# bentherien/point-cloud-reid

Hardware: AMD Instinct MI355X
Metric: siamese pair-comparisons/sec @1024 pts (higher is better)
Workload: dtype bf16x3

## Files before the change

### point-cloud-reid_amd/csrc/attn_kernels_impl.h

```cpp
#pragma once
#ifndef PCR_ATTN_PREC
#define PCR_ATTN_PREC 0
#endif
#include "tile_dense.h"

#include <stdio.h>

#include <vector>

namespace {
constexpr int kAPrec = PCR_ATTN_PREC;
struct AttnArgs {
  pcr_attn_params p;
  int dbg;
  int wpc;
};

constexpr int kATraceWgs = 512, kATraceRecs = 24, kATraceMarks = 8;
__device__ unsigned long long g_attn_trace[2 * kATraceWgs * kATraceRecs * kATraceMarks];


__device__ __forceinline__ void pos_hidden(float *dst, int RP, const float *P, const float *w0,
                                           const float *b0, int d, int T) {
  for (int e = threadIdx.x; e < d * T; e += blockDim.x) {
// ... 636 lines not shown
        for (int s2 = 0; s2 < 2; s2++) {
          float xv[8];
#pragma unroll
          for (int e = 0; e < 8; e++) xv[e] = xf[8 * s2 + e];
          bf_split8(xv, ah[s2], al[s2], true);
        }
        f32x16 acc[2];
#pragma unroll
        for (int cb = 0; cb < 2; cb++)
#pragma unroll
          for (int r = 0; r < 16; r++) acc[cb][r] = 0.f;
        const bf16x8 *wb = reinterpret_cast<const bf16x8 *>(s_w) + lane;
#pragma unroll
        for (int s2 = 0; s2 < 4; s2++) {
          bf16x8 wh[2], wl[2];
#pragma unroll
          for (int cb = 0; cb < 2; cb++) {
            wh[cb] = wb[((s2 * 2 + cb) * 2) * 64];
            wl[cb] = wb[((s2 * 2 + cb) * 2 + 1) * 64];
          }
#pragma unroll
          for (int cb = 0; cb < 2; cb++) acc[cb] = __builtin_amdgcn_mfma_f32_32x32x16_bf16(ah[s2], wh[cb], acc[cb], 0, 0, 0);
#pragma unroll
          for (int cb = 0; cb < 2; cb++) acc[cb] = __builtin_amdgcn_mfma_f32_32x32x16_bf16(al[s2], wh[cb], acc[cb], 0, 0, 0);
#pragma unroll
          for (int cb = 0; cb < 2; cb++) acc[cb] = __builtin_amdgcn_mfma_f32_32x32x16_bf16(ah[s2], wl[cb], acc[cb], 0, 0, 0);
        }
#pragma unroll
        for (int r = 0; r < 16; r++) {
          acc[0][r] = elu1(acc[0][r] + bias0);
          acc[1][r] = (acc[1][r] + bias1) * inv_sk;
          ks += acc[0][r];
        }
#pragma unroll
        for (int r = 0; r < 16; r++) kv = __builtin_amdgcn_mfma_f32_32x32x2f32(acc[0][r], acc[1][r], kv, 0, 0, 0);
      }
    }
    ks += __shfl_xor(ks, 32, 64);
    float *KVl = s_red + cslot * KVS, *s_kt = KVl + D * LD;
    for (int round = 0; round < wpc2; round++) {
      if (wsub == round) {
#pragma unroll
        for (int r = 0; r < 16; r++) {
          float *dst = KVl + ((r & 3) + 8 * (r >> 2) + 4 * h) * LD + j;
          *dst = round == 0 ? kv[r] : *dst + kv[r];
        }
        if (h == 0) s_kt[j] = round == 0 ? ks : s_kt[j] + ks;
      }
      __syncthreads();
    }
    if (live && wsub == 0) {
      float *kvo = p.kv + (size_t)b * ((size_t)D * D + D);
      const float *ap = s_wm + j * LD + h;
      const float *bp = KVl + j * LD + h;
      const int hd = j / dh;
      f32x16 m;
#pragma unroll
      for (int r = 0; r < 16; r++) m[r] = 0.f;
#pragma unroll 4
      for (int s2 = 0; s2 < 16; s2++) {
        const float bv = bp[2 * s2];
        m = __builtin_amdgcn_mfma_f32_32x32x2f32((2 * s2 + h) / dh == hd ? bv : 0.f, ap[2 * s2], m, 0, 0, 0);
      }
      bf16x8 *img = reinterpret_cast<bf16x8 *>(kvo);
#pragma unroll
      for (int G = 0; G < 2; G++) {
        float v[8];
#pragma unroll
        for (int e = 0; e < 8; e++) v[e] = m[8 * G + e];
        bf16x8 hi, lo;
        bf_split8(v, hi, lo, true);
        const size_t unit = (((size_t)G * (D >> 5)) * 2) * 64 + h * 32 + j;
        img[unit] = hi;
        img[unit + 64] = lo;
      }
      if (lane < D) kvo[(size_t)D * D + lane] = s_kt[lane];
    }
    __syncthreads();
  }
}
#endif

__global__ __launch_bounds__(kThreads) void attn_kv_fold_kernel(AttnArgs a) {
  extern __shared__ __attribute__((aligned(16))) float smem[];
  const pcr_attn_params &p = a.p;
  const int d = p.d, dh = d / p.nhead, ld = d + 1, nsplit = p.kv_splits, tid = threadIdx.x;
  const size_t b = blockIdx.x, per = (size_t)d * d + d;
  float *KVl = smem, *s_kt = smem + d * ld;
  const float *part = p.kv_part + b * nsplit * per;
  for (int e = tid; e < d * d + d; e += kThreads) {
    float v = part[e];
    for (int y = 1; y < nsplit; y++) v += part[(size_t)y * per + e];
    if (e < d * d) {
      const int dd = e / d, c = e - dd * d;
      KVl[dd * ld + c] = (dd / dh == c / dh) ? v : 0.f;
    } else {
      s_kt[e - d * d] = v;
    }
  }
  __syncthreads();
  attn_kv_fold_write(p, KVl, s_kt, b);
}

#if PCR_ATTN_PREC == 0
template <int NRW>
__global__ __launch_bounds__(kThreads) void attn_kv_wide_kernel(AttnArgs a) {
  constexpr int TB = 1, T = 32, RP = 33, BAND = 64, RPK = BAND + 1;
  extern __shared__ __attribute__((aligned(16))) float smem[];
  const pcr_attn_params &p = a.p;
  const int d = p.d, c2 = p.c2, dh = d / p.nhead;
  const int g = blockIdx.x, hd = (g * BAND) / dh;
  const int OPW = BAND + dh;
  float *XH = smem;
  float *KB = XH, *VB = XH + BAND * RP;
  float *P = XH + (c2 + d) * RP;
  float *s_w0 = P + 3 * RP, *s_b0 = s_w0 + 3 * d;
  float *s_ks = s_b0 + d;
  const int tid = threadIdx.x, lane = tid & 63, wave = tid >> 6;
  const int l31 = lane & 31, h = lane >> 5;
  const size_t b = blockIdx.y;
  for (int e = tid; e < 3 * d; e += kThreads) s_w0[e] = p.pos0_w[e];
  for (int e = tid; e < d; e += kThreads) s_b0[e] = p.pos0_b[e];
  const float *feat = p.feat_k + b * c2 * p.Sk;
  const float *xyz = p.xyz_k + b * p.Sk * 3;
  const float sk = (float)p.Sk;
  const float *wband = p.wkv_wide + (size_t)g * ((size_t)ceil8(c2 + d) * OPW);
  const float *bband = p.bkv_wide + (size_t)g * OPW;
  const int nj = dh >> 5, nT = 2 * nj;
  f32x16 acc[4];
#pragma unroll
  for (int i = 0; i < 4; i++)
#pragma unroll
    for (int r = 0; r < 16; r++) acc[i][r] = 0.f;
  const int krow = tid & (BAND - 1), kpart = tid >> 6;
  float ksum = 0.f;
  for (int t0 = 0; t0 < p.Sk; t0 += T) {
    const int valid = p.Sk - t0;
    load_tile(XH, RP, feat, c2, c2, p.Sk, t0, T);
    load_xyz3(P, RP, xyz, p.Sk, t0, T);
    __syncthreads();
    pos_hidden(XH + c2 * RP, RP, P, s_w0, s_b0, d, T);
    __syncthreads();
    tile_dense2<TB, NRW, 0, true>(XH, c2 + d, wband, OPW, true,
                                  [&](const f32x16 &acc, int cb, int tb, int l31, int h) {
      const int t = tb * 32 + l31;
      float *dst = XH + (cb * 32 + 4 * h) * RP + t;
      const bool live = t < valid;
      if (cb * 32 < BAND) {
#pragma unroll
        for (int r = 0; r < 16; r++) dst[((r & 3) + 8 * (r >> 2)) * RP] = live ? elu1(acc[r]) : 0.f;
      } else {
#pragma unroll
        for (int r = 0; r < 16; r++) dst[((r & 3) + 8 * (r >> 2)) * RP] = live ? acc[r] / sk : 0.f;
      }
    }, bband);
    __syncthreads();
    {
      const float *row = KB + krow * RP;
      for (int t = kpart; t < T; t += 4) ksum += row[t];
    }
#pragma unroll
    for (int it = 0; it < 4; it++) {
      const int item = wave + 4 * it;
      if (item < nT) {
        const int ib = item / nj, jb = item - ib * nj;
        const float *ap = KB + (ib * 32 + l31) * RP + h;
        const float *bp = VB + (jb * 32 + l31) * RP + h;
#pragma unroll 4
        for (int ks = 0; ks < T / 2; ks++)
          acc[it] = __builtin_amdgcn_mfma_f32_32x32x2f32(ap[2 * ks], bp[2 * ks], acc[it], 0, 0, 0);
      }
    }
    __syncthreads();
  }
  float *KVt = smem;
  s_ks[tid] = ksum;
  __syncthreads();
  const float ks_total = tid < BAND ? s_ks[tid] + s_ks[64 + tid] + s_ks[128 + tid] + s_ks[192 + tid] : 0.f;
  __syncthreads();
#pragma unroll
  for (int it = 0; it < 4; it++) {
    const int item = wave + 4 * it;
    if (item < nT) {
      const int ib = item / nj, jb = item - ib * nj;
      const int v = jb * 32 + l31;
#pragma unroll
      for (int r = 0; r < 16; r++) KVt[v * RPK + ib * 32 + (r & 3) + 8 * (r >> 2) + 4 * h] = acc[it][r];
    }
  }
  __syncthreads();
  float *kv = p.kv + b * ((size_t)d * d + d);
  if (tid < BAND) kv[(size_t)d * d + g * BAND + tid] = ks_total;
  const float *wm = p.wmerge_packed + (size_t)(hd * dh / 8) * d * 8;
  tile_dense(KVt, dh, RPK, 2, wm, d, [&](float m, int o, int t) {
    const int dd = g * BAND + t;
    const int kb = dd >> 3, rem = dd & 7;
    kv[(((size_t)kb * d + o) * 2 + (rem & 1)) * 4 + (rem >> 1)] = m;
  });
}

#endif

template <int TB, int NR>
__global__ __launch_bounds__(kThreads) void attn_apply_kernel(AttnArgs a) {
  constexpr int T = 32 * TB, RP = T + 1;
  extern __shared__ __attribute__((aligned(16))) float smem[];
  const pcr_attn_params &p = a.p;
  const int d = p.d, c1 = p.c1, cout = p.cout;
  const int catC = c1 + d, catP = ceil8(catC);
  int rowsU = catP > 2 * d ? catP : 2 * d;
  if (ceil32(cout) > rowsU) rowsU = ceil32(cout);
  if (ceil32(p.cfinal) > rowsU) rowsU = ceil32(p.cfinal);
  float *U = smem;
  float *P = U + rowsU * RP;
  float *zs = P + 3 * RP;
  float *red = zs + p.nhead * RP;
  float *cst = red + 2 * (kThreads / T) * T;
  float *s_ksum = cst, *s_ln1g = cst + d, *s_ln1b = cst + 2 * d, *s_ln2g = cst + 3 * d, *s_ln2b = s_ln2g + cout;
  float *s_w0 = s_ln2b + cout, *s_b0 = s_w0 + 3 * d;
  const int tid = threadIdx.x;
  const size_t b = blockIdx.y;
  const int t0 = blockIdx.x * T;
  const size_t bq_ = p.q_index ? (size_t)p.q_index[b] : b;
  const float *feat = p.feat_q + bq_ * c1 * p.Lq;
  const size_t kb_ = p.kv_index ? (size_t)p.kv_index[b] : b;
  const float *kv = p.kv + kb_ * ((size_t)d * d + d);
  const int dh = d / p.nhead;
  for (int e = tid; e < d; e += kThreads) {
    s_ksum[e] = kv[(size_t)d * d + e];
    s_ln1g[e] = p.ln1_g[e];
    s_ln1b[e] = p.ln1_b[e];
    if (p.q_pos) {
      s_w0[3 * e] = p.pos0_w[3 * e];
      s_w0[3 * e + 1] = p.pos0_w[3 * e + 1];
      s_w0[3 * e + 2] = p.pos0_w[3 * e + 2];
      s_b0[e] = p.pos0_b[e];
    }
  }
  for (int e = tid; e < cout; e += kThreads) {
    s_ln2g[e] = p.ln2_g[e];
    s_ln2b[e] = p.ln2_b[e];
  }
  const float *ksum = s_ksum;
  float *MSG = U + c1 * RP;

  load_tile(U, RP, feat, c1, c1, p.Lq, t0, T);
  if (p.q_pos) {
    load_xyz3(P, RP, p.xyz_q + bq_ * p.Lq * 3, p.Lq, t0, T);
    __syncthreads();
    pos_hidden(MSG, RP, P, s_w0, s_b0, d, T);
    for (int e = tid; e < (catP - catC) * T; e += kThreads) U[(catC + e / T) * RP + e % T] = 0.f;
  } else {
    for (int e = tid; e < (catP - c1) * T; e += kThreads) U[(c1 + e / T) * RP + e % T] = 0.f;
  }
  __syncthreads();
  tile_dense2p<kAPrec, TB, NR>(U, p.q_pos ? catP : ceil8(c1), p.wq, d, true,
                               [&](float v, int o, int t) { MSG[o * RP + t] = elu1(v); }, p.bq);
  __syncthreads();
  for (int e = tid; e < p.nhead * T; e += kThreads) {
    const int hd = e / T, t = e - hd * T;
    float z = 0.f;
    for (int c = 0; c < dh; c++) z += MSG[(hd * dh + c) * RP + t] * ksum[hd * dh + c];
    zs[hd * RP + t] = (1.0f / (z + 1e-6f)) * (float)p.Sk;
  }
  __syncthreads();
  for (int hd = 0; hd < p.nhead; hd++)
    for (int e = tid; e < dh * T; e += kThreads) {
      const int o = hd * dh + e / T, t = e % T;
      MSG[o * RP + t] *= zs[hd * RP + t];
    }
  __syncthreads();
  tile_dense2p<kAPrec, TB, NR>(MSG, d, kv, d, true, [&](float v, int o, int t) { MSG[o * RP + t] = v; });
  __syncthreads();
  tile_layernorm(MSG, d, RP, T, s_ln1g, s_ln1b, red);
  tile_dense2p<kAPrec, TB, NR>(U, catP, p.wmlp0, 2 * d, true, [&](float v, int o, int t) { U[o * RP + t] = fmaxf(v, 0.f); });
  __syncthreads();
  tile_dense2p<kAPrec, TB, NR>(U, 2 * d, p.wmlp2, ceil32(cout), true, [&](float v, int o, int t) { U[o * RP + t] = v; });
  __syncthreads();
  tile_layernorm(U, cout, RP, T, s_ln2g, s_ln2b, red);
  if (p.residual) {
    for (int e = tid; e < cout * T; e += kThreads) {
      const int c = e / T, t = e - c * T;
      if (t0 + t < p.Lq) U[c * RP + t] += feat[(size_t)c * p.Lq + t0 + t];
    }
    __syncthreads();
  }
  int cres = cout;
  if (p.cfinal) {
    const int cf = p.cfinal;
    tile_dense2p<kAPrec, TB, NR>(U, cout, p.wfinal, ceil32(cf), true, [&](float v, int o, int t) { U[o * RP + t] = v; },
                                 p.bfinal);
    __syncthreads();
    cres = cf;
  }
  float *out = p.out + b * cres * p.Lq;
  for (int e = tid; e < cres * T; e += kThreads) {
    const int c = e / T, t = e - c * T;
    if (t0 + t < p.Lq) out[(size_t)c * p.Lq + t0 + t] = U[c * RP + t];
  }
}

#if PCR_ATTN_PREC != 0
constexpr int kApsWaves = 8;
template <bool QPOS, int C1S, int CF, int NOB = 2, int ND = 2, bool POOL = false>
__global__ __launch_bounds__(64 * kApsWaves) __attribute__((amdgpu_waves_per_eu(2, 2)))
void attn_apply_stream64_kernel(AttnArgs a) {
  static_assert(!QPOS || C1S == 2 * ND, "q_pos needs c1 == d");
  static_assert(NOB <= 2 || (NOB == 4 && !CF), "cout = 128 has no trailing conv");
  static_assert(!POOL || (!CF && NOB == 2), "pooled output: cout = 64, no trailing conv");
  constexpr int D = 32 * ND, SD = 2 * ND;
  constexpr int SQ = C1S + (QPOS ? SD : 0), S0 = C1S + SD, NX = 8 * C1S;
  extern __shared__ __attribute__((aligned(16))) float smem[];
  const pcr_attn_params &p = a.p;
  bf16x8 *s_wq = reinterpret_cast<bf16x8 *>(smem);
  bf16x8 *s_w0 = s_wq + SQ * ND * 128;
  bf16x8 *s_w2 = s_w0 + S0 * ND * 256;
  float *s_c = reinterpret_cast<float *>(s_w2 + ND * NOB * 512);
  f32x4 *s_p0 = reinterpret_cast<f32x4 *>(s_c + 448);
  float *s_ks = reinterpret_cast<float *>(s_p0 + 64);
  const int tid = threadIdx.x, lane = tid & 63, j = lane & 31, h = lane >> 5;
  const int wave = __builtin_amdgcn_readfirstlane(tid >> 6);
  {
    const f32x4 *wq = reinterpret_cast<const f32x4 *>(p.wq),
                *w0 = reinterpret_cast<const f32x4 *>((p.c1 & 15) ? p.wmlp0_bf_xpad : p.wmlp0),
                *w2 = reinterpret_cast<const f32x4 *>(p.wmlp2);
    f32x4 *dq = reinterpret_cast<f32x4 *>(s_wq), *d0 = reinterpret_cast<f32x4 *>(s_w0), *d2 = reinterpret_cast<f32x4 *>(s_w2);
    for (int e = tid; e < SQ * ND * 128; e += 64 * kApsWaves) dq[e] = wq[e];
    for (int e = tid; e < S0 * ND * 256; e += 64 * kApsWaves) d0[e] = w0[e];
    for (int e = tid; e < ND * NOB * 512; e += 64 * kApsWaves) d2[e] = w2[e];
    if (tid < D) {
      s_c[tid] = p.bq[tid];
      s_c[64 + tid] = p.ln1_g[tid];
      s_c[128 + tid] = p.ln1_b[tid];

      if (QPOS) s_p0[tid] = f32x4{p.pos0_w[3 * tid], p.pos0_w[3 * tid + 1], p.pos0_w[3 * tid + 2], p.pos0_b[tid]};
    }
    if (tid < 32 * NOB) {
      s_c[192 + tid] = p.ln2_g[tid];
      s_c[192 + 32 * NOB + tid] = p.ln2_b[tid];
    }
    if (CF && tid < 32 * CF) s_c[320 + tid] = p.bfinal[tid];
  }
  __syncthreads();
  const int nblk = p.Lq >> 5;
  const long nitem = (long)p.B * nblk;
  const int dh = D / p.nhead;
  const float skf = (float)p.Sk;
  float *ksw = s_ks + wave * 64;
  auto cvec = [&](const float *base, int cb, int g) __attribute__((always_inline)) {
    return *reinterpret_cast<const f32x4 *>(base + 32 * cb + 8 * g + 4 * h);
  };
  auto to_ops = [&](const f32x16 &acc, int G, bf16x8 &oh, bf16x8 &ol) __attribute__((always_inline)) {
    float v[8];
#pragma unroll
    for (int e = 0; e < 8; e++) v[e] = acc[8 * G + e];
    bf_split8(v, oh, ol, true);
  };
#ifdef PCR_SA_TRACE_BUILD
  const bool tracing = (a.dbg & 256) && lane == 0 && (wave == 0 || wave == 5) && blockIdx.x < kATraceWgs;
  unsigned long long *trace = g_attn_trace + (size_t)(2 * blockIdx.x + (wave ? 1 : 0)) * (kATraceRecs * kATraceMarks);
  int trace_it = 0;
#define PCR_AMARK(m)                                                                                       \
  do {                                                                                                     \
    if (tracing && trace_it < kATraceRecs) trace[trace_it * kATraceMarks + (m)] = __builtin_readcyclecounter(); \
  } while (0)
#define PCR_ANEXT() trace_it++
#else
#define PCR_AMARK(m) do { } while (0)
#define PCR_ANEXT() do { } while (0)
#endif
  const long nwav = (long)gridDim.x * kApsWaves, gw = (long)blockIdx.x * kApsWaves + wave;
  long pc = gw;
  int pblk = 0;
  float pmax = -INFINITY, psum = 0.f;
  for (long it = gw; POOL ? pc < p.B : it < nitem; it += POOL ? 0 : nwav) {
    asm volatile("" ::: "memory");
    PCR_AMARK(0);
    const long b = POOL ? pc : it / nblk;
    const int blk = POOL ? pblk : (int)(it - b * nblk);
    const size_t bq_ = p.q_index ? (size_t)p.q_index[b] : (size_t)b;
    const size_t kb_ = p.kv_index ? (size_t)p.kv_index[b] : (size_t)b;
    const float *kvp = p.kv + kb_ * ((size_t)D * D + D);
    const int t = blk * 32 + j;
    const __amdgpu_buffer_rsrc_t rfeat = __builtin_amdgcn_make_buffer_rsrc(
        const_cast<float *>(p.feat_q + bq_ * p.c1 * p.Lq), 0, p.c1 * p.Lq * 4, 0x00020000);
    const int vo = (4 * h * p.Lq + t) * 4;
    float xf[NX];
#pragma unroll
    for (int e = 0; e < NX; e++) {
      const int ch = 16 * (e >> 3) + bf_kpos(0, e & 7);
      xf[e] = __builtin_bit_cast(float, __builtin_amdgcn_raw_buffer_load_b32(rfeat, vo, ch * p.Lq * 4, 0));
    }
    if (lane < D) ksw[lane] = kvp[(size_t)D * D + lane];
    bf16x8 bh[4 * ND], bl[4 * ND];
    if constexpr (QPOS) {
      const float *xyz = p.xyz_q + (bq_ * p.Lq + t) * 3;
      const float px = xyz[0], py = xyz[1], pz = xyz[2];
#pragma unroll
      for (int s2 = 0; s2 < SD; s2++) {
        float hv[8];
#pragma unroll
        for (int e = 0; e < 8; e++) {
          const f32x4 w = s_p0[16 * s2 + bf_kpos(0, e) + 4 * h];
          const float v = w[0] * px + w[1] * py + w[2] * pz + w[3];
          hv[e] = relu_i(v);
        }
        bf_split8(hv, bh[C1S + s2], bl[C1S + s2], true);
      }
    }
#pragma unroll
    for (int e = 0; e < NX; e++) asm volatile("" : "+v"(xf[e]));
#pragma unroll
    for (int s2 = 0; s2 < C1S; s2++) {
      float xv[8];
#pragma unroll
      for (int e = 0; e < 8; e++) xv[e] = xf[8 * s2 + e];
      bf_split8(xv, bh[s2], bl[s2], true);
    }
    PCR_AMARK(1);
    f32x16 q[ND];
#pragma unroll
    for (int cb = 0; cb < ND; cb++)
#pragma unroll
      for (int r = 0; r < 16; r++) q[cb][r] = 0.f;
    {
      const bf16x8 *wb = s_wq + lane;
#pragma unroll
      for (int s2 = 0; s2 < SQ; s2++) {
        bf16x8 wh[ND], wl[ND];
#pragma unroll
        for (int cb = 0; cb < ND; cb++) {
          wh[cb] = wb[((s2 * ND + cb) * 2) * 64];
          wl[cb] = wb[((s2 * ND + cb) * 2 + 1) * 64];
        }
#pragma unroll
        for (int cb = 0; cb < ND; cb++) q[cb] = __builtin_amdgcn_mfma_f32_32x32x16_bf16(wh[cb], bh[s2], q[cb], 0, 0, 0);
#pragma unroll
        for (int cb = 0; cb < ND; cb++) q[cb] = __builtin_amdgcn_mfma_f32_32x32x16_bf16(wh[cb], bl[s2], q[cb], 0, 0, 0);
#pragma unroll
        for (int cb = 0; cb < ND; cb++) q[cb] = __builtin_amdgcn_mfma_f32_32x32x16_bf16(wl[cb], bh[s2], q[cb], 0, 0, 0);
      }
    }
    PCR_AMARK(2);
    bf16x8 mh[SD][ND], ml[SD][ND];
    {
      const bf16x8 *mb = reinterpret_cast<const bf16x8 *>(kvp) + lane;
#pragma unroll
      for (int s2 = 0; s2 < SD; s2++)
#pragma unroll
        for (int cb = 0; cb < ND; cb++) {
          mh[s2][cb] = mb[((s2 * ND + cb) * 2) * 64];
          ml[s2][cb] = mb[((s2 * ND + cb) * 2 + 1) * 64];
        }
    }
    __builtin_amdgcn_fence(__ATOMIC_RELEASE, "wavefront");
    __builtin_amdgcn_wave_barrier();
    __builtin_amdgcn_fence(__ATOMIC_ACQUIRE, "wavefront");
    float z16[2][2] = {{0.f, 0.f}, {0.f, 0.f}};
#pragma unroll
    for (int cb = 0; cb < ND; cb++)
#pragma unroll
      for (int g = 0; g < 4; g++) {
        const f32x4 bqv = cvec(s_c, cb, g), ksv = cvec(ksw, cb, g);
        float zz = 0.f;
#pragma unroll
        for (int qq = 0; qq < 4; qq++) {
          const float v = elu1(q[cb][4 * g + qq] + bqv[qq]);
          q[cb][4 * g + qq] = v;
          zz += v * ksv[qq];
        }
        if ((g & 1) == 0) z16[cb][g >> 1] = zz;
        else z16[cb][g >> 1] += zz;
      }
    float zs[2][2];
    {
      float za = z16[0][0], zb = z16[0][1], zc = z16[1][0], zd = z16[1][1];
      if (dh >= 32) {
        za += zb; zb = za;
        zc += zd; zd = zc;
      }
      if (ND == 2 && dh >= 64) {
        za += zc; zb = za; zc = za; zd = za;
      }
      za += __shfl_xor(za, 32, 64);
      zb += __shfl_xor(zb, 32, 64);
      zc += __shfl_xor(zc, 32, 64);
      zd += __shfl_xor(zd, 32, 64);
      zs[0][0] = (1.0f / (za + 1e-6f)) * skf;
      zs[0][1] = (1.0f / (zb + 1e-6f)) * skf;
      zs[1][0] = (1.0f / (zc + 1e-6f)) * skf;
      zs[1][1] = (1.0f / (zd + 1e-6f)) * skf;
    }
#pragma unroll
    for (int cb = 0; cb < ND; cb++)
#pragma unroll
      for (int r = 0; r < 16; r++) q[cb][r] *= zs[cb][r >> 3];
    bf16x8 ch_[SD], cl_[SD];
#pragma unroll
    for (int cb = 0; cb < ND; cb++)
#pragma unroll
      for (int G = 0; G < 2; G++) to_ops(q[cb], G, ch_[2 * cb + G], cl_[2 * cb + G]);
    f32x16 m[ND];
#pragma unroll
    for (int cb = 0; cb < ND; cb++)
#pragma unroll
      for (int r = 0; r < 16; r++) m[cb][r] = 0.f;
#pragma unroll
    for (int s2 = 0; s2 < SD; s2++) {
#pragma unroll
      for (int cb = 0; cb < ND; cb++) m[cb] = __builtin_amdgcn_mfma_f32_32x32x16_bf16(mh[s2][cb], ch_[s2], m[cb], 0, 0, 0);
#pragma unroll
      for (int cb = 0; cb < ND; cb++) m[cb] = __builtin_amdgcn_mfma_f32_32x32x16_bf16(mh[s2][cb], cl_[s2], m[cb], 0, 0, 0);
#pragma unroll
      for (int cb = 0; cb < ND; cb++) m[cb] = __builtin_amdgcn_mfma_f32_32x32x16_bf16(ml[s2][cb], ch_[s2], m[cb], 0, 0, 0);
    }
    auto layernorm = [&](auto &v, auto nb_tag, const float *gam, const float *bet) __attribute__((always_inline)) {
      constexpr int NB = decltype(nb_tag)::value;
      float sm = 0.f;
#pragma unroll
      for (int cb = 0; cb < NB; cb++)
#pragma unroll
        for (int r = 0; r < 16; r++) sm += v[cb][r];
      sm += __shfl_xor(sm, 32, 64);
      const float mean = sm / (32.0f * NB);
      float vr = 0.f;
#pragma unroll
      for (int cb = 0; cb < NB; cb++)
#pragma unroll
        for (int r = 0; r < 16; r++) {
          const float dlt = v[cb][r] - mean;
          vr += dlt * dlt;
        }
      vr += __shfl_xor(vr, 32, 64);
      const float inv = 1.0f / sqrtf(vr / (32.0f * NB) + 1e-5f);
#pragma unroll
      for (int cb = 0; cb < NB; cb++)
#pragma unroll
        for (int g = 0; g < 4; g++) {
          const f32x4 gv = cvec(gam, cb, g), bv = cvec(bet, cb, g);
#pragma unroll
          for (int qq = 0; qq < 4; qq++) v[cb][4 * g + qq] = (v[cb][4 * g + qq] - mean) * inv * gv[qq] + bv[qq];
        }
    };
    PCR_AMARK(3);
    layernorm(m, std::integral_constant<int, ND>{}, s_c + 64, s_c + 128);
    PCR_AMARK(4);
#pragma unroll
    for (int s2 = 0; s2 < C1S; s2++) {
      float xv[8];
#pragma unroll
      for (int e = 0; e < 8; e++) xv[e] = xf[8 * s2 + e];
      bf_split8(xv, bh[s2], bl[s2], true);
    }
#pragma unroll
    for (int cb = 0; cb < ND; cb++)
#pragma unroll
      for (int G = 0; G < 2; G++) to_ops(m[cb], G, bh[C1S + 2 * cb + G], bl[C1S + 2 * cb + G]);
    f32x16 f[SD];
#pragma unroll
    for (int cb = 0; cb < SD; cb++)
#pragma unroll
      for (int r = 0; r < 16; r++) f[cb][r] = 0.f;
    {
      const bf16x8 *wb = s_w0 + lane;
#pragma unroll
      for (int s2 = 0; s2 < S0; s2++) {
        bf16x8 wh[SD], wl[SD];
#pragma unroll
        for (int cb = 0; cb < SD; cb++) {
          wh[cb] = wb[((s2 * SD + cb) * 2) * 64];
          wl[cb] = wb[((s2 * SD + cb) * 2 + 1) * 64];
        }
#pragma unroll
        for (int cb = 0; cb < SD; cb++) f[cb] = __builtin_amdgcn_mfma_f32_32x32x16_bf16(wh[cb], bh[s2], f[cb], 0, 0, 0);
#pragma unroll
        for (int cb = 0; cb < SD; cb++) f[cb] = __builtin_amdgcn_mfma_f32_32x32x16_bf16(wh[cb], bl[s2], f[cb], 0, 0, 0);
#pragma unroll
        for (int cb = 0; cb < SD; cb++) f[cb] = __builtin_amdgcn_mfma_f32_32x32x16_bf16(wl[cb], bh[s2], f[cb], 0, 0, 0);
      }
    }
#pragma unroll
    for (int cb = 0; cb < SD; cb++) {
#pragma unroll
      for (int r = 0; r < 16; r++) f[cb][r] = relu_i(f[cb][r]);
#pragma unroll
      for (int G = 0; G < 2; G++) to_ops(f[cb], G, bh[2 * cb + G], bl[2 * cb + G]);
    }
    PCR_AMARK(5);
    f32x16 o[NOB];
#pragma unroll
    for (int cb = 0; cb < NOB; cb++)
#pragma unroll
      for (int r = 0; r < 16; r++) o[cb][r] = 0.f;
    {
      const bf16x8 *wb = s_w2 + lane;
#pragma unroll
      for (int s2 = 0; s2 < 4 * ND; s2++) {
        bf16x8 wh[NOB], wl[NOB];
#pragma unroll
        for (int cb = 0; cb < NOB; cb++) {
          wh[cb] = wb[((s2 * NOB + cb) * 2) * 64];
          wl[cb] = wb[((s2 * NOB + cb) * 2 + 1) * 64];
        }
#pragma unroll
        for (int cb = 0; cb < NOB; cb++) o[cb] = __builtin_amdgcn_mfma_f32_32x32x16_bf16(wh[cb], bh[s2], o[cb], 0, 0, 0);
#pragma unroll
        for (int cb = 0; cb < NOB; cb++) o[cb] = __builtin_amdgcn_mfma_f32_32x32x16_bf16(wh[cb], bl[s2], o[cb], 0, 0, 0);
#pragma unroll
        for (int cb = 0; cb < NOB; cb++) o[cb] = __builtin_amdgcn_mfma_f32_32x32x16_bf16(wl[cb], bh[s2], o[cb], 0, 0, 0);
      }
    }
    PCR_AMARK(6);
    layernorm(o, std::integral_constant<int, NOB>{}, s_c + 192, s_c + 192 + 32 * NOB);
    if constexpr (C1S == 2 * NOB) {
      if (p.residual) {
#pragma unroll
        for (int cb = 0; cb < NOB; cb++)
#pragma unroll
          for (int r = 0; r < 16; r++) o[cb][r] += xf[16 * cb + r];
      }
    }
    if constexpr (POOL) {
      float vm[16], vs[16];
      {
        const bool up = (j & 1) != 0;
#pragma unroll
        for (int r = 0; r < 16; r++) {
          const float lo_ = o[r >> 4][r & 15], hi_ = o[(r + 16) >> 4][(r + 16) & 15];
          const float tk = up ? hi_ : lo_, uk = up ? lo_ : hi_;
          const float pu = __uint_as_float(pcr_sort_partner<2, 1>(__float_as_uint(uk), lane));
          vm[r] = fmaxf(tk, pu);
          vs[r] = tk + pu;
        }
      }
#define PCR_POOL_STEP(N, J, BIT)                                                                      \
      {                                                                                               \
        const bool up = (j & BIT) != 0;                                                               \
        _Pragma("unroll") for (int r = 0; r < N; r++) {                                               \
          const float tm = up ? vm[r + N] : vm[r], um = up ? vm[r] : vm[r + N];                       \
          const float ts = up ? vs[r + N] : vs[r], us = up ? vs[r] : vs[r + N];                       \
          vm[r] = fmaxf(tm, __uint_as_float(pcr_sort_partner<2 * J, J>(__float_as_uint(um), lane)));  \
          vs[r] = ts + __uint_as_float(pcr_sort_partner<2 * J, J>(__float_as_uint(us), lane));        \
        }                                                                                             \
      }
      PCR_POOL_STEP(8, 2, 2)
      PCR_POOL_STEP(4, 4, 4)
      PCR_POOL_STEP(2, 8, 8)
      PCR_POOL_STEP(1, 16, 16)
#undef PCR_POOL_STEP
      pmax = fmaxf(pmax, vm[0]);
      psum += vs[0];
      if (++pblk == nblk) {
        const int e = ((j & 1) << 4) | ((j & 2) << 2) | (j & 4) | ((j & 8) >> 2) | ((j & 16) >> 4);
        const int ch = 16 * (e >> 3) + bf_kpos(h, e & 7);
        float *po = p.pool_out + (size_t)b * 128;
        po[ch] = pmax;
        po[64 + ch] = psum;
        pmax = -INFINITY;
        psum = 0.f;
        pblk = 0;
        pc += nwav;
      }
    } else if constexpr (!CF) {
      const __amdgpu_buffer_rsrc_t rout =
          __builtin_amdgcn_make_buffer_rsrc(p.out + (size_t)b * (32 * NOB) * p.Lq, 0, 32 * NOB * p.Lq * 4, 0x00020000);
#pragma unroll
      for (int e = 0; e < 16 * NOB; e++) {
        const int ch = 16 * (e >> 3) + bf_kpos(0, e & 7);
        const float v = o[e >> 4][e & 15];
        __builtin_amdgcn_raw_buffer_store_b32(__builtin_bit_cast(unsigned, v), rout, vo, ch * p.Lq * 4, 0);
      }
    } else {
#pragma unroll
      for (int cb = 0; cb < NOB; cb++)
#pragma unroll
        for (int G = 0; G < 2; G++) to_ops(o[cb], G, bh[2 * cb + G], bl[2 * cb + G]);
      f32x16 fo[CF ? CF : 1];
#pragma unroll
      for (int cb = 0; cb < CF; cb++)
#pragma unroll
        for (int r = 0; r < 16; r++) fo[cb][r] = 0.f;
      const bf16x8 *wb = reinterpret_cast<const bf16x8 *>(p.wfinal) + lane;
#pragma unroll
      for (int s2 = 0; s2 < 2 * NOB; s2++) {
        bf16x8 wh[CF ? CF : 1], wl[CF ? CF : 1];
#pragma unroll
        for (int cb = 0; cb < CF; cb++) {
          wh[cb] = wb[((s2 * CF + cb) * 2) * 64];
          wl[cb] = wb[((s2 * CF + cb) * 2 + 1) * 64];
        }
#pragma unroll
        for (int cb = 0; cb < CF; cb++) fo[cb] = __builtin_amdgcn_mfma_f32_32x32x16_bf16(wh[cb], bh[s2], fo[cb], 0, 0, 0);
#pragma unroll
        for (int cb = 0; cb < CF; cb++) fo[cb] = __builtin_amdgcn_mfma_f32_32x32x16_bf16(wh[cb], bl[s2], fo[cb], 0, 0, 0);
#pragma unroll
        for (int cb = 0; cb < CF; cb++) fo[cb] = __builtin_amdgcn_mfma_f32_32x32x16_bf16(wl[cb], bh[s2], fo[cb], 0, 0, 0);
      }
      const __amdgpu_buffer_rsrc_t rout =
          __builtin_amdgcn_make_buffer_rsrc(p.out + (size_t)b * (32 * CF) * p.Lq, 0, 32 * CF * p.Lq * 4, 0x00020000);
#pragma unroll
      for (int cb = 0; cb < CF; cb++)
#pragma unroll
        for (int g = 0; g < 4; g++) {
          const f32x4 bv = cvec(s_c + 320, cb, g);
#pragma unroll
          for (int qq = 0; qq < 4; qq++) {
            const int e = 16 * cb + 4 * g + qq;
            const int ch = 16 * (e >> 3) + bf_kpos(0, e & 7);
            const float v = fo[cb][4 * g + qq] + bv[qq];
            __builtin_amdgcn_raw_buffer_store_b32(__builtin_bit_cast(unsigned, v), rout, vo, ch * p.Lq * 4, 0);
          }
        }
    }
    __builtin_amdgcn_wave_barrier();
    PCR_AMARK(7);
    PCR_ANEXT();
  }
#undef PCR_AMARK
#undef PCR_ANEXT
}

template <int NB, bool TRANS = false>
__device__ __forceinline__ void ap128_step(f32x16 (&acc)[NB], const bf16x8 *wb, int ls, const bf16x8 &bh, const bf16x8 &bl) {
  auto mm = [](const bf16x8 &w, const bf16x8 &x, const f32x16 &c) __attribute__((always_inline)) {
    return TRANS ? __builtin_amdgcn_mfma_f32_32x32x16_bf16(x, w, c, 0, 0, 0) : __builtin_amdgcn_mfma_f32_32x32x16_bf16(w, x, c, 0, 0, 0);
  };
#pragma unroll
  for (int c0 = 0; c0 < NB; c0 += 4) {
    bf16x8 wh[4], wl[4];
#pragma unroll
    for (int cb = 0; cb < 4; cb++) {
      wh[cb] = wb[((ls * NB + c0 + cb) * 2) * 64];
      wl[cb] = wb[((ls * NB + c0 + cb) * 2 + 1) * 64];
    }
#pragma unroll
    for (int cb = 0; cb < 4; cb++) acc[c0 + cb] = mm(wh[cb], bh, acc[c0 + cb]);
#pragma unroll
    for (int cb = 0; cb < 4; cb++) acc[c0 + cb] = mm(wh[cb], bl, acc[c0 + cb]);
#pragma unroll
    for (int cb = 0; cb < 4; cb++) acc[c0 + cb] = mm(wl[cb], bh, acc[c0 + cb]);
    asm volatile("" ::: "memory");
  }
}
constexpr int kAp128Waves = 4, kAp128ChunkU = 2048, kAp128Chunks = 16;
constexpr int kAp128Npc = kAp128ChunkU / (64 * kAp128Waves);
__device__ __forceinline__ void ring128_fetch(f32x4 (&stg)[kAp128Npc], __amdgpu_buffer_rsrc_t r, int kk, int tid) {
#pragma unroll
  for (int u = 0; u < kAp128Npc; u++)
    stg[u] = __builtin_bit_cast(f32x4, __builtin_amdgcn_raw_buffer_load_b128(r, tid * 16, (kk * kAp128ChunkU + u * 64 * kAp128Waves) * 16, 0));
  asm volatile("" ::: "memory");
}
__device__ __forceinline__ void ring128_commit(f32x4 *s_ring, const f32x4 (&stg)[kAp128Npc], int k, int tid) {
  f32x4 *dst = s_ring + (k & 1) * kAp128ChunkU + tid;
#pragma unroll
  for (int u = 0; u < kAp128Npc; u++) dst[u * 64 * kAp128Waves] = stg[u];
  __syncthreads();
}
constexpr size_t kAp128Lds = (size_t)2 * kAp128ChunkU * 16 + (640 + 4 * 128 + kAp128Waves * 128) * sizeof(float);
template <int NH>
__global__ __launch_bounds__(64 * kAp128Waves) __attribute__((amdgpu_waves_per_eu(1, 1)))
void attn_apply_stream128_kernel(AttnArgs a) {
  constexpr int D = 128, ND = 4, SD = 8, GPH = 8 / NH;
  extern __shared__ __attribute__((aligned(16))) float smem[];
  const pcr_attn_params &p = a.p;
  f32x4 *s_ring = reinterpret_cast<f32x4 *>(smem);
  int coff = 2 * kAp128ChunkU * 4;
  asm volatile("" : "+s"(coff));
  float *s_c = smem + coff;
  f32x4 *s_p0 = reinterpret_cast<f32x4 *>(s_c + 640);
  float *s_ks = s_c + 640 + 4 * 128;
  const int tid = threadIdx.x, lane = tid & 63, j = lane & 31, h = lane >> 5;
  const int wave = __builtin_amdgcn_readfirstlane(tid >> 6);
  const __amdgpu_buffer_rsrc_t rwq = __builtin_amdgcn_make_buffer_rsrc(const_cast<float *>(p.wq), 0, 4 * kAp128ChunkU * 16, 0x00020000),
                               rw0 = __builtin_amdgcn_make_buffer_rsrc(const_cast<float *>(p.wmlp0), 0, 8 * kAp128ChunkU * 16, 0x00020000),
                               rw2 = __builtin_amdgcn_make_buffer_rsrc(const_cast<float *>(p.wmlp2), 0, 4 * kAp128ChunkU * 16, 0x00020000);
  f32x4 stg[kAp128Npc];
  auto fetch = [&](int k) __attribute__((always_inline)) {
    k %= kAp128Chunks;
    ring128_fetch(stg, k < 4 ? rwq : (k < 12 ? rw0 : rw2), k < 4 ? k : (k < 12 ? k - 4 : k - 12), tid);
  };
  auto commit = [&](int k) __attribute__((always_inline)) { ring128_commit(s_ring, stg, k, tid); };
  for (int e = tid; e < D; e += 64 * kAp128Waves) {
    s_c[e] = p.bq[e];
    s_c[128 + e] = p.ln1_g[e];
    s_c[256 + e] = p.ln1_b[e];
    s_c[384 + e] = p.ln2_g[e];
    s_c[512 + e] = p.ln2_b[e];
    s_p0[e] = f32x4{p.pos0_w[3 * e], p.pos0_w[3 * e + 1], p.pos0_w[3 * e + 2], p.pos0_b[e]};
  }
  fetch(0);
  commit(0);
  const int nblk = p.Lq >> 5;
  const long nitem = (long)p.B * nblk;
  const float skf = (float)p.Sk;
  float *ksw = s_ks + wave * 128;
  auto cvec = [&](const float *base, int cb, int g) __attribute__((always_inline)) {
    return *reinterpret_cast<const f32x4 *>(base + 32 * cb + 8 * g + 4 * h);
  };
  auto to_ops = [&](const f32x16 &acc, int G, bf16x8 &oh, bf16x8 &ol) __attribute__((always_inline)) {
    float v[8];
#pragma unroll
    for (int e = 0; e < 8; e++) v[e] = acc[8 * G + e];
    bf_split8(v, oh, ol, true);
  };
  auto layernorm = [&](f32x16 (&v)[ND], const float *gam, const float *bet) __attribute__((always_inline)) {
    float sm = 0.f;
#pragma unroll
    for (int cb = 0; cb < ND; cb++)
#pragma unroll
      for (int r = 0; r < 16; r++) sm += v[cb][r];
    sm += __shfl_xor(sm, 32, 64);
    const float mean = sm / (float)D;
    float vr = 0.f;
#pragma unroll
    for (int cb = 0; cb < ND; cb++)
#pragma unroll
      for (int r = 0; r < 16; r++) {
        const float dlt = v[cb][r] - mean;
        vr += dlt * dlt;
      }
    vr += __shfl_xor(vr, 32, 64);
    const float inv = 1.0f / sqrtf(vr / (float)D + 1e-5f);
#pragma unroll
    for (int cb = 0; cb < ND; cb++)
#pragma unroll
      for (int g = 0; g < 4; g++) {
        const f32x4 gv = cvec(gam, cb, g), bv = cvec(bet, cb, g);
#pragma unroll
        for (int qq = 0; qq < 4; qq++) v[cb][4 * g + qq] = (v[cb][4 * g + qq] - mean) * inv * gv[qq] + bv[qq];
      }
  };
  for (long it0 = (long)blockIdx.x * kAp128Waves; it0 < nitem; it0 += (long)gridDim.x * kAp128Waves) {
    const long item = it0 + wave;
    const bool live = item < nitem;
    const long it = live ? item : nitem - 1;
    const long b = it / nblk;
    const int blk = (int)(it - b * nblk);
    const size_t bq_ = p.q_index ? (size_t)p.q_index[b] : (size_t)b;
    const size_t kb_ = p.kv_index ? (size_t)p.kv_index[b] : (size_t)b;
    const float *kvp = p.kv + kb_ * ((size_t)D * D + D);
    const int t = blk * 32 + j;
    const __amdgpu_buffer_rsrc_t rfeat = __builtin_amdgcn_make_buffer_rsrc(
        const_cast<float *>(p.feat_q + bq_ * D * p.Lq), 0, D * p.Lq * 4, 0x00020000);
    const int vo = (4 * h * p.Lq + t) * 4;
    auto load_x = [&](float (&xf)[64]) __attribute__((always_inline)) {
#pragma unroll
      for (int e = 0; e < 64; e++) {
        const int ch = 16 * (e >> 3) + bf_kpos(0, e & 7);
        xf[e] = __builtin_bit_cast(float, __builtin_amdgcn_raw_buffer_load_b32(rfeat, vo, ch * p.Lq * 4, 0));
      }
    };
    ksw[lane] = kvp[(size_t)D * D + lane];
    ksw[64 + lane] = kvp[(size_t)D * D + 64 + lane];
    bf16x8 bh[16], bl[16];
    {
      float xf[64];
      load_x(xf);
      const float *xyz = p.xyz_q + (bq_ * p.Lq + t) * 3;
      const float px = xyz[0], py = xyz[1], pz = xyz[2];
#pragma unroll
      for (int s2 = 0; s2 < SD; s2++) {
        float hv[8];
#pragma unroll
        for (int e = 0; e < 8; e++) {
          const f32x4 w = s_p0[16 * s2 + bf_kpos(0, e) + 4 * h];
          const float v = w[0] * px + w[1] * py + w[2] * pz + w[3];
          hv[e] = relu_i(v);
        }
        bf_split8(hv, bh[SD + s2], bl[SD + s2], true);
      }
#pragma unroll
      for (int e = 0; e < 64; e++) asm volatile("" : "+v"(xf[e]));
#pragma unroll
      for (int s2 = 0; s2 < SD; s2++) {
        float xv[8];
#pragma unroll
        for (int e = 0; e < 8; e++) xv[e] = xf[8 * s2 + e];
        bf_split8(xv, bh[s2], bl[s2], true);
      }
    }
    f32x16 q[ND];
#pragma unroll
    for (int cb = 0; cb < ND; cb++)
#pragma unroll
      for (int g = 0; g < 4; g++) {
        const f32x4 bqv = cvec(s_c, cb, g);
#pragma unroll
        for (int qq = 0; qq < 4; qq++) q[cb][4 * g + qq] = bqv[qq];
      }
#pragma unroll
    for (int k = 0; k < 4; k++) {
      fetch(k + 1);
      const bf16x8 *wb = reinterpret_cast<const bf16x8 *>(s_ring + (k & 1) * kAp128ChunkU) + lane;
#pragma unroll
      for (int ls = 0; ls < 4; ls++) ap128_step<ND>(q, wb, ls, bh[4 * k + ls], bl[4 * k + ls]);
      commit(k + 1);
    }
    float zg[SD];
#pragma unroll
    for (int cb = 0; cb < ND; cb++)
#pragma unroll
      for (int g = 0; g < 4; g++) {
        const f32x4 ksv = cvec(ksw, cb, g);
        float zz = 0.f;
#pragma unroll
        for (int qq = 0; qq < 4; qq++) {
          const float v = elu1(q[cb][4 * g + qq]);
          q[cb][4 * g + qq] = v;
          zz += v * ksv[qq];
        }
        if ((g & 1) == 0) zg[2 * cb + (g >> 1)] = zz;
        else zg[2 * cb + (g >> 1)] += zz;
      }
    float zs[NH];
#pragma unroll
    for (int hd = 0; hd < NH; hd++) {
      float z = zg[hd * GPH];
#pragma unroll
      for (int gi = 1; gi < GPH; gi++) z += zg[hd * GPH + gi];
      z += __shfl_xor(z, 32, 64);
      zs[hd] = (1.0f / (z + 1e-6f)) * skf;
    }
// ... 620 lines not shown
```

Before: 66360.

## Software-pipeline next item's feature loads across iterations in stream64 attention kernel

Result: no change. 66190 (-0.2%).

```diff
diff --git a/point-cloud-reid_amd/csrc/attn_kernels_impl.h b/point-cloud-reid_amd/csrc/attn_kernels_impl.h
--- a/point-cloud-reid_amd/csrc/attn_kernels_impl.h
+++ b/point-cloud-reid_amd/csrc/attn_kernels_impl.h
@@ -962,6 +962,12 @@
 
 #if PCR_ATTN_PREC != 0
 constexpr int kApsWaves = 8;
+#ifndef PCR_APS_V
+#define PCR_APS_V 1
+#endif
+#ifndef PCR_APS_M_EARLY
+#define PCR_APS_M_EARLY 1
+#endif
 template <bool QPOS, int C1S, int CF, int NOB = 2, int ND = 2, bool POOL = false>
 __global__ __launch_bounds__(64 * kApsWaves) __attribute__((amdgpu_waves_per_eu(2, 2)))
 void attn_apply_stream64_kernel(AttnArgs a) {
@@ -1007,8 +1013,10 @@
   const int dh = D / p.nhead;
   const float skf = (float)p.Sk;
   float *ksw = s_ks + wave * 64;
+  int clane = (int)(s_c - smem) + 4 * h;
+  asm volatile("" : "+v"(clane));
   auto cvec = [&](const float *base, int cb, int g) __attribute__((always_inline)) {
-    return *reinterpret_cast<const f32x4 *>(base + 32 * cb + 8 * g + 4 * h);
+    return *reinterpret_cast<const f32x4 *>(smem + clane + ((int)(base - s_c) + 32 * cb + 8 * g));
   };
   auto to_ops = [&](const f32x16 &acc, int G, bf16x8 &oh, bf16x8 &ol) __attribute__((always_inline)) {
     float v[8];
@@ -1033,29 +1041,68 @@
   long pc = gw;
   int pblk = 0;
   float pmax = -INFINITY, psum = 0.f;
+  float xf[NX], ks_n = 0.f, px_n = 0.f, py_n = 0.f, pz_n = 0.f;
+  long b_n = 0;
+  size_t bq_n = 0, kb_n = 0;
+  int vo_n = 0;
+  const float *kvp_n = p.kv;
+  __amdgpu_buffer_rsrc_t rfeat_n = __builtin_amdgcn_make_buffer_rsrc(const_cast<float *>(p.feat_q), 0, 0, 0x00020000);
+  typedef const __attribute__((address_space(4))) int *cint_ptr;
+  auto lookup = [&](long b) __attribute__((always_inline)) {
+    bq_n = p.q_index ? (size_t)((cint_ptr)p.q_index)[b] : (size_t)b;
+    kb_n = p.kv_index ? (size_t)((cint_ptr)p.kv_index)[b] : (size_t)b;
+    b_n = b;
+  };
+  auto request = [&](int blk) __attribute__((always_inline)) {
+    kvp_n = p.kv + kb_n * ((size_t)D * D + D);
+    const int t = blk * 32 + j;
+    rfeat_n = __builtin_amdgcn_make_buffer_rsrc(
+        const_cast<float *>(p.feat_q + bq_n * p.c1 * p.Lq), 0, p.c1 * p.Lq * 4, 0x00020000);
+    vo_n = (4 * h * p.Lq + t) * 4;
+    if constexpr (QPOS) {
+      const float *xyz = p.xyz_q + (bq_n * p.Lq + t) * 3;
+      px_n = xyz[0], py_n = xyz[1], pz_n = xyz[2];
+    }
+#pragma unroll
+    for (int e = 0; e < NX; e++) {
+      const int ch = 16 * (e >> 3) + bf_kpos(0, e & 7);
+      xf[e] = __builtin_bit_cast(float, __builtin_amdgcn_raw_buffer_load_b32(rfeat_n, vo_n, ch * p.Lq * 4, 0));
+    }
+    if (lane < D) ks_n = kvp_n[(size_t)D * D + lane];
+  };
+  const long wq = nwav / nblk;
+  const int wr = (int)(nwav - wq * nblk);
+  int blk_n = 0;
+  if (POOL ? pc < p.B : gw < nitem) {
+    const long b0 = POOL ? pc : gw / nblk;
+    blk_n = POOL ? 0 : (int)(gw - b0 * nblk);
+    lookup(b0);
+    request(blk_n);
+  }
   for (long it = gw; POOL ? pc < p.B : it < nitem; it += POOL ? 0 : nwav) {
     asm volatile("" ::: "memory");
     PCR_AMARK(0);
-    const long b = POOL ? pc : it / nblk;
-    const int blk = POOL ? pblk : (int)(it - b * nblk);
-    const size_t bq_ = p.q_index ? (size_t)p.q_index[b] : (size_t)b;
-    const size_t kb_ = p.kv_index ? (size_t)p.kv_index[b] : (size_t)b;
-    const float *kvp = p.kv + kb_ * ((size_t)D * D + D);
-    const int t = blk * 32 + j;
-    const __amdgpu_buffer_rsrc_t rfeat = __builtin_amdgcn_make_buffer_rsrc(
-        const_cast<float *>(p.feat_q + bq_ * p.c1 * p.Lq), 0, p.c1 * p.Lq * 4, 0x00020000);
-    const int vo = (4 * h * p.Lq + t) * 4;
-    float xf[NX];
-#pragma unroll
-    for (int e = 0; e < NX; e++) {
-      const int ch = 16 * (e >> 3) + bf_kpos(0, e & 7);
-      xf[e] = __builtin_bit_cast(float, __builtin_amdgcn_raw_buffer_load_b32(rfeat, vo, ch * p.Lq * 4, 0));
-    }
-    if (lane < D) ksw[lane] = kvp[(size_t)D * D + lane];
+    const long b = b_n;
+    const float *kvp = kvp_n;
+    [[maybe_unused]] const __amdgpu_buffer_rsrc_t rfeat = rfeat_n;
+    const int vo = vo_n;
+    const float ks = ks_n;
+    [[maybe_unused]] const int blk_c = blk_n;
+    if constexpr (POOL) {
+      const bool last = pblk + 1 == nblk;
+      const long nb = last && pc + nwav < p.B ? pc + nwav : pc;
+      blk_n = last ? (nb == pc ? pblk : 0) : pblk + 1;
+      lookup(nb);
+    } else {
+      long nb = b + wq;
+      blk_n = blk_c + wr;
+      if (blk_n >= nblk) blk_n -= nblk, nb++;
+      if (nb >= p.B) nb = b, blk_n = blk_c;
+      lookup(nb);
+    }
     bf16x8 bh[4 * ND], bl[4 * ND];
     if constexpr (QPOS) {
-      const float *xyz = p.xyz_q + (bq_ * p.Lq + t) * 3;
-      const float px = xyz[0], py = xyz[1], pz = xyz[2];
+      const float px = px_n, py = py_n, pz = pz_n;
 #pragma unroll
       for (int s2 = 0; s2 < SD; s2++) {
         float hv[8];
@@ -1078,6 +1125,18 @@
       bf_split8(xv, bh[s2], bl[s2], true);
     }
     PCR_AMARK(1);
+    bf16x8 mh[SD][ND], ml[SD][ND];
+    auto request_m = [&]() __attribute__((always_inline)) {
+      const bf16x8 *mb = reinterpret_cast<const bf16x8 *>(kvp) + lane;
+#pragma unroll
+      for (int s2 = 0; s2 < SD; s2++)
+#pragma unroll
+        for (int cb = 0; cb < ND; cb++) {
+          mh[s2][cb] = mb[((s2 * ND + cb) * 2) * 64];
+          ml[s2][cb] = mb[((s2 * ND + cb) * 2 + 1) * 64];
+        }
+    };
+    if constexpr (PCR_APS_M_EARLY) request_m();
     f32x16 q[ND];
 #pragma unroll
     for (int cb = 0; cb < ND; cb++)
@@ -1102,17 +1161,8 @@
       }
     }
     PCR_AMARK(2);
-    bf16x8 mh[SD][ND], ml[SD][ND];
-    {
-      const bf16x8 *mb = reinterpret_cast<const bf16x8 *>(kvp) + lane;
-#pragma unroll
-      for (int s2 = 0; s2 < SD; s2++)
-#pragma unroll
-        for (int cb = 0; cb < ND; cb++) {
-          mh[s2][cb] = mb[((s2 * ND + cb) * 2) * 64];
-          ml[s2][cb] = mb[((s2 * ND + cb) * 2 + 1) * 64];
-        }
-    }
+    if constexpr (!PCR_APS_M_EARLY) request_m();
+    if (lane < D) ksw[lane] = ks;
     __builtin_amdgcn_fence(__ATOMIC_RELEASE, "wavefront");
     __builtin_amdgcn_wave_barrier();
     __builtin_amdgcn_fence(__ATOMIC_ACQUIRE, "wavefront");
@@ -1203,19 +1253,14 @@
         }
     };
     PCR_AMARK(3);
+    if constexpr ((PCR_APS_V & 4) != 0) __builtin_amdgcn_sched_barrier(0);
     layernorm(m, std::integral_constant<int, ND>{}, s_c + 64, s_c + 128);
     PCR_AMARK(4);
 #pragma unroll
-    for (int s2 = 0; s2 < C1S; s2++) {
-      float xv[8];
-#pragma unroll
-      for (int e = 0; e < 8; e++) xv[e] = xf[8 * s2 + e];
-      bf_split8(xv, bh[s2], bl[s2], true);
-    }
-#pragma unroll
     for (int cb = 0; cb < ND; cb++)
 #pragma unroll
       for (int G = 0; G < 2; G++) to_ops(m[cb], G, bh[C1S + 2 * cb + G], bl[C1S + 2 * cb + G]);
+    if constexpr ((PCR_APS_V & 2) != 0) __builtin_amdgcn_sched_barrier(0);
     f32x16 f[SD];
 #pragma unroll
     for (int cb = 0; cb < SD; cb++)
@@ -1247,6 +1292,20 @@
       for (int G = 0; G < 2; G++) to_ops(f[cb], G, bh[2 * cb + G], bl[2 * cb + G]);
     }
     PCR_AMARK(5);
+    __builtin_amdgcn_sched_barrier(0);
+    constexpr bool RES = C1S == 2 * NOB;
+    [[maybe_unused]] float xr[RES ? NX : 1];
+    if constexpr (RES) {
+      if (p.residual) {
+#pragma unroll
+        for (int e = 0; e < NX; e++) {
+          const int ch = 16 * (e >> 3) + bf_kpos(0, e & 7);
+          xr[e] = __builtin_bit_cast(float, __builtin_amdgcn_raw_buffer_load_b32(rfeat, vo, ch * p.Lq * 4, 0));
+        }
+      }
+    }
+    request(blk_n);
+    if constexpr ((PCR_APS_V & 1) != 0) __builtin_amdgcn_sched_barrier(0);
     f32x16 o[NOB];
 #pragma unroll
     for (int cb = 0; cb < NOB; cb++)
@@ -1272,12 +1331,12 @@
     }
     PCR_AMARK(6);
     layernorm(o, std::integral_constant<int, NOB>{}, s_c + 192, s_c + 192 + 32 * NOB);
-    if constexpr (C1S == 2 * NOB) {
+    if constexpr (RES) {
       if (p.residual) {
 #pragma unroll
         for (int cb = 0; cb < NOB; cb++)
 #pragma unroll
-          for (int r = 0; r < 16; r++) o[cb][r] += xf[16 * cb + r];
+          for (int r = 0; r < 16; r++) o[cb][r] += xr[16 * cb + r];
       }
     }
     if constexpr (POOL) {
```
